# chen-bowen/instacart_next_order_recommendation

Hardware: AMD Instinct MI355X
Metric: recommend_qps_top20_49k7_catalog (higher is better)
Workload: dtype f16x3 (f32 operands split into 2 f16 planes, 3 f16 MFMAs per product, f32 accumulate; fp32-level accuracy)

## Files before the change

### instacart_next_order_recommendation_amd/csrc/encoder.hip

```cpp
#include <stdlib.h>

#include <mutex>
#include <type_traits>
#include <vector>

#include "common.h"
#include "gemm_x3.h"
#include "wt_gemm.h"
#include "encoder_x3.h"

namespace icrec {

__device__ __forceinline__ int find_seq(const int32_t* __restrict__ cu, int n_seqs, int t) {
    int lo = 0, hi = n_seqs;
    while (hi - lo > 1) {
        int mid = (lo + hi) >> 1;
        if (cu[mid] <= t) lo = mid; else hi = mid;
    }
    return lo;
}

template <int H, bool SPLIT>
__device__ __forceinline__ void ln_row(float (&v)[H / 64], const float* __restrict__ g, const float* __restrict__ b,
                                       float eps, float* __restrict__ out, _Float16* __restrict__ oh,
                                       _Float16* __restrict__ ol, int lane) {
    float s = 0.0f;
#pragma unroll
    for (int j = 0; j < H / 64; ++j) s = s + v[j];
    const float mean = wave_sum_f32(s) / (float)H;
    float q = 0.0f;
#pragma unroll
    for (int j = 0; j < H / 64; ++j) {
        float d = v[j] - mean;
        q = fmaf(d, d, q);
    }
    const float var = wave_sum_f32(q) / (float)H;
    const float rstd = 1.0f / sqrtf(var + eps);
#pragma unroll
    for (int j = 0; j < H / 64; ++j) {
        const int i = lane + 64 * j;
        const float y = fmaf((v[j] - mean) * rstd, g[i], b[i]);
        if (SPLIT) {
            _Float16 hi, lo;
            split_act(y, hi, lo);
            oh[i] = hi;
            ol[i] = lo;
        } else {
            out[i] = y;
        }
    }
}

template <int H, bool SPLIT>
__global__ __launch_bounds__(256) void embed_ln_kernel(const int32_t* __restrict__ ids,
                                                       const int32_t* __restrict__ cu, int n_seqs, int T,
                                                       const float* __restrict__ word, const float* __restrict__ pos,
                                                       const float* __restrict__ type, const float* __restrict__ g,
                                                       const float* __restrict__ b, float eps, int vocab, int max_pos,
                                                       float* __restrict__ x, _Float16* __restrict__ xh,
                                                       _Float16* __restrict__ xl) {
    const int lane = threadIdx.x & 63;
    const int t = blockIdx.x * 4 + (threadIdx.x >> 6);
    if (t >= T) return;
    const int s = find_seq(cu, n_seqs, t);
    int id = ids[t];
    id = id < 0 ? 0 : (id >= vocab ? vocab - 1 : id);
    int p = t - cu[s];
    p = p >= max_pos ? max_pos - 1 : p;
    float v[H / 64];
#pragma unroll
    for (int j = 0; j < H / 64; ++j) {
        const int i = lane + 64 * j;
        v[j] = (word[(size_t)id * H + i] + type[i]) + pos[(size_t)p * H + i];
    }
    ln_row<H, SPLIT>(v, g, b, eps, x + (size_t)t * H, xh + (size_t)t * H, xl + (size_t)t * H, lane);
}

template <int H, bool SPLIT>
__global__ __launch_bounds__(256) void add_ln_kernel(const float* __restrict__ a, float* __restrict__ x, int T,
                                                     const float* __restrict__ g, const float* __restrict__ b,
                                                     float eps, _Float16* __restrict__ xh,
                                                     _Float16* __restrict__ xl) {
    const int lane = threadIdx.x & 63;
    const int t = blockIdx.x * 4 + (threadIdx.x >> 6);
    if (t >= T) return;
    float v[H / 64];
#pragma unroll
    for (int j = 0; j < H / 64; ++j) {
        const int i = lane + 64 * j;
        v[j] = a[(size_t)t * H + i] + x[(size_t)t * H + i];
    }
    ln_row<H, SPLIT>(v, g, b, eps, x + (size_t)t * H, xh + (size_t)t * H, xl + (size_t)t * H, lane);
}

__device__ __forceinline__ float gelu_erf(float x) { return x * 0.5f * (1.0f + erff(x * 0.70710678118654752440f)); }

template <class Cfg, bool GELU>
__global__ __launch_bounds__(Cfg::THREADS, 2) void linear_kernel(const float* __restrict__ A, int M, int K,
                                                                 const float* __restrict__ W, int N,
                                                                 const float* __restrict__ bias,
                                                                 float* __restrict__ out, int n_tiles_n) {
    __shared__ __attribute__((aligned(16))) float smem[Cfg::LDS_FLOATS];
    float* As = smem;
    float* Bs = smem + Cfg::BM * LDK;
    const int lane = threadIdx.x & 63, wave = threadIdx.x >> 6;
    const int wm = wave / Cfg::WAVES_N, wn = wave % Cfg::WAVES_N;
    const int bid = xcd_remap(blockIdx.x, gridDim.x);
    const int mt = bid / n_tiles_n, nt = bid % n_tiles_n;
    const int64_t m0 = (int64_t)mt * Cfg::BM, n0 = (int64_t)nt * Cfg::BN;
    TileRegs<Cfg> pre;
    f32x16 acc[Cfg::TM][Cfg::TN];
    tile_gemm<Cfg>(acc, A, m0, M, W, n0, N, K, As, Bs, pre, false);
#pragma unroll
    for (int j = 0; j < Cfg::TN; ++j) {
        const int64_t col = n0 + (wn * Cfg::TN + j) * 32 + (lane & 31);
        const float bv = col < N ? bias[col] : 0.0f;
#pragma unroll
        for (int i = 0; i < Cfg::TM; ++i)
#pragma unroll
            for (int e = 0; e < 16; ++e) {
                const int64_t row = m0 + (wm * Cfg::TM + i) * 32 + acc_row(e, lane);
                if (row < M && col < N) {
                    float v = acc[i][j][e] + bv;
                    if (GELU) v = gelu_erf(v);
                    out[row * N + col] = v;
                }
            }
    }
}

constexpr int DH = 32;
constexpr int LDQ = 36;

template <int NKT, int WAVES, bool SPLIT>
__global__ __launch_bounds__(WAVES * 64) void attention_kernel(const float* __restrict__ qkv,
                                                               const int32_t* __restrict__ cu, int heads, int H,
                                                               float scale_log2e, float* __restrict__ ctx,
                                                               _Float16* __restrict__ ch, _Float16* __restrict__ cl) {
    __shared__ __attribute__((aligned(16))) float Ks[NKT * 32 * LDQ];
    __shared__ __attribute__((aligned(16))) float Vs[NKT * 32 * DH];
    __shared__ float Ls[WAVES * 32];

    const int tid = threadIdx.x, lane = tid & 63, wave = tid >> 6;
    const int s = blockIdx.x / heads, hd = blockIdx.x % heads;
    const int t0 = cu[s], L = cu[s + 1] - t0;
    const int nkt = (L + 31) >> 5;
    if (nkt > NKT || (NKT > 1 && nkt <= NKT / 2)) return;
    const int qb0 = blockIdx.y * WAVES;
    if (qb0 >= nkt) return;
    const int ld = 3 * H;

    for (int id = tid; id < nkt * 32 * 8; id += WAVES * 64) {
        const int row = id >> 3, c = id & 7;
        const int rr = row < L ? row : L - 1;
        const float* src = qkv + (size_t)(t0 + rr) * ld + hd * DH + c * 4;
        const float4 kv = *reinterpret_cast<const float4*>(src + H);
        const float4 vv = *reinterpret_cast<const float4*>(src + 2 * H);
        float* kp = Ks + row * LDQ + (c >> 1) * 8 + (c & 1) * 2;
        *reinterpret_cast<float2*>(kp) = make_float2(kv.x, kv.z);
        *reinterpret_cast<float2*>(kp + 4) = make_float2(kv.y, kv.w);
        *reinterpret_cast<float4*>(Vs + row * DH + c * 4) = vv;
    }
    const int r = lane & 31, h = lane >> 5;
    const int qb = qb0 + wave;
    float4 qf[4];
    {
        int qr = qb * 32 + r;
        qr = qr < L ? qr : L - 1;
        const float4* qp = reinterpret_cast<const float4*>(qkv + (size_t)(t0 + qr) * ld + hd * DH);
#pragma unroll
        for (int kq = 0; kq < 4; ++kq) {
            const float4 a = qp[2 * kq], b = qp[2 * kq + 1];
            qf[kq] = h == 0 ? make_float4(a.x, a.z, b.x, b.z) : make_float4(a.y, a.w, b.y, b.w);
        }
    }
    __syncthreads();
    if (qb >= nkt) return;

    f32x16 sc[NKT];
#pragma unroll
    for (int kt = 0; kt < NKT; ++kt) {
#pragma unroll
        for (int e = 0; e < 16; ++e) sc[kt][e] = 0.0f;
        if (kt < nkt) {
#pragma unroll
            for (int kq = 0; kq < 4; ++kq) {
                const float4 kf = *reinterpret_cast<const float4*>(Ks + (kt * 32 + r) * LDQ + kq * 8 + h * 4);
                sc[kt] = __builtin_amdgcn_mfma_f32_32x32x2f32(kf.x, qf[kq].x, sc[kt], 0, 0, 0);
                sc[kt] = __builtin_amdgcn_mfma_f32_32x32x2f32(kf.y, qf[kq].y, sc[kt], 0, 0, 0);
                sc[kt] = __builtin_amdgcn_mfma_f32_32x32x2f32(kf.z, qf[kq].z, sc[kt], 0, 0, 0);
                sc[kt] = __builtin_amdgcn_mfma_f32_32x32x2f32(kf.w, qf[kq].w, sc[kt], 0, 0, 0);
            }
        }
    }
    float mx = -INFINITY;
#pragma unroll
    for (int kt = 0; kt < NKT; ++kt) {
        if (kt < nkt) {
            const bool last = kt == nkt - 1;
#pragma unroll
            for (int e = 0; e < 16; ++e) {
                float v = sc[kt][e] * scale_log2e;
                if (last && kt * 32 + acc_row(e, lane) >= L) v = -INFINITY;
                sc[kt][e] = v;
                mx = fmaxf(mx, v);
            }
        }
    }
    mx = fmaxf(mx, __shfl_xor(mx, 32, 64));
    float lsum = 0.0f;
#pragma unroll
    for (int kt = 0; kt < NKT; ++kt) {
        if (kt < nkt) {
#pragma unroll
            for (int e = 0; e < 16; ++e) {
                const float p = __builtin_amdgcn_exp2f(sc[kt][e] - mx);
                sc[kt][e] = p;
                lsum = lsum + p;
            }
        }
    }
    {
        const float other = __shfl_xor(lsum, 32, 64);
        lsum = h == 0 ? lsum + other : other + lsum;
    }
    if (h == 0) Ls[wave * 32 + r] = lsum;
    f32x16 o;
#pragma unroll
    for (int e = 0; e < 16; ++e) o[e] = 0.0f;
#pragma unroll
    for (int kt = 0; kt < NKT; ++kt) {
        if (kt < nkt) {
#pragma unroll
            for (int e = 0; e < 16; ++e) {
                const int key = kt * 32 + (e & 3) + 8 * (e >> 2) + 4 * h;
                o = __builtin_amdgcn_mfma_f32_32x32x2f32(sc[kt][e], Vs[key * DH + r], o, 0, 0, 0);
            }
        }
    }
#pragma unroll
    for (int e = 0; e < 16; ++e) {
        const int qrow = acc_row(e, lane);
        const int tq = qb * 32 + qrow;
        if (tq < L) {
            const float v = o[e] / Ls[wave * 32 + qrow];
            const size_t at = (size_t)(t0 + tq) * H + hd * DH + r;
            if (SPLIT) {
                _Float16 hi, lo;
                split_act(v, hi, lo);
                ch[at] = hi;
                cl[at] = lo;
            } else {
                ctx[at] = v;
            }
        }
    }
}

__global__ __launch_bounds__(1024) void seq_order_kernel(const int32_t* __restrict__ cu, int n_seqs,
                                                         int32_t* __restrict__ order) {
    __shared__ int hist[257];
    const int tid = threadIdx.x;
    for (int i = tid; i < 257; i += 1024) hist[i] = 0;
    __syncthreads();
    for (int s0 = tid; s0 < n_seqs; s0 += 1024) {
        const int s = n_seqs - 1 - s0;
        int L = cu[s + 1] - cu[s];
        L = L < 1 ? 1 : (L > 256 ? 256 : L);
        atomicAdd(&hist[256 - ((L + 31) & ~31)], 1);
    }
    __syncthreads();
    if (tid == 0) {
        int run = 0;
        for (int b = 0; b < 257; ++b) { const int c = hist[b]; hist[b] = run; run += c; }
    }
    __syncthreads();
    for (int s0 = tid; s0 < n_seqs; s0 += 1024) {
        const int s = n_seqs - 1 - s0;
        int L = cu[s + 1] - cu[s];
        L = L < 1 ? 1 : (L > 256 ? 256 : L);
        order[atomicAdd(&hist[256 - ((L + 31) & ~31)], 1)] = s;
    }
}

typedef _Float16 half2v __attribute__((ext_vector_type(2)));

__device__ __forceinline__ void split8(const float (&x)[8], half8& hi, half8& lo) {
#pragma unroll
    for (int j = 0; j < 8; ++j) {
        const _Float16 a = (_Float16)x[j];
        hi[j] = a;
        lo[j] = (_Float16)((x[j] - (float)a) * LO_SCALE);
    }
}

__device__ __forceinline__ half4 lds_read_tr(const _Float16* p) {
    typedef __fp16 fp16x4 __attribute__((__vector_size__(4 * sizeof(__fp16))));
    return __builtin_bit_cast(half4, __builtin_amdgcn_ds_read_tr16_b64_v4f16(
                                         (__attribute__((address_space(3))) fp16x4*)(reinterpret_cast<uintptr_t>(p))));
}

template <int NKT, int WAVES, bool SPLIT>
__global__ __launch_bounds__(WAVES * 64, (NKT >= 6 ? 4 : NKT == 4 ? 3 : 1)) void attention_x3_kernel(const float* __restrict__ qkv,
                                                                  const int32_t* __restrict__ cu, int heads, int H,
                                                                  float scale_log2e, float* __restrict__ ctx,
                                                                  _Float16* __restrict__ ch, _Float16* __restrict__ cl,
                                                                  const int32_t* __restrict__ order, int nlo) {
    constexpr bool RECOMP = NKT >= 6;
    __shared__ __attribute__((aligned(16))) _Float16 Kbuf[2 * NKT * 32 * 32];
    _Float16* const Kh = Kbuf;
    _Float16* const Kl = Kbuf + NKT * 32 * 32;
    __shared__ __attribute__((aligned(16))) _Float16 Vh[NKT * 32 * 32];
    __shared__ __attribute__((aligned(16))) _Float16 Vl[NKT * 32 * 32];
    __shared__ float Ls[WAVES * 32];
    constexpr bool OB = SPLIT;
    static_assert(!OB || WAVES * 2 * 32 * 32 <= 2 * NKT * 32 * 32, "the output tiles reuse the K planes");
    _Float16* const Ob = Kbuf;

    const int tid = threadIdx.x, lane = tid & 63, wave = tid >> 6;
    const int sidx = blockIdx.x / heads, hd = blockIdx.x % heads;
    const int s = order != nullptr ? order[sidx] : sidx;
    const int t0 = cu[s], L = cu[s + 1] - t0;
    const int nkt = (L + 31) >> 5;
    if (nkt > NKT || nkt <= nlo) return;
    const int qb0 = blockIdx.y * WAVES;
    if (qb0 >= nkt) return;
    const int ld = 3 * H;

    const int r = lane & 31, h = lane >> 5;
    const int qb = qb0 + wave;
    ICREC_STAMP(0, 0);
    half8 qh[2], ql[2];
    {
        int qr = qb * 32 + r;
        qr = qr < L ? qr : L - 1;
        const float* qp = qkv + (size_t)(t0 + qr) * ld + hd * DH;
#pragma unroll
        for (int ks = 0; ks < 2; ++ks) {
            const f32x4 a = *reinterpret_cast<const f32x4*>(qp + 16 * ks + 8 * h);
            const f32x4 b = *reinterpret_cast<const f32x4*>(qp + 16 * ks + 8 * h + 4);
            half4 ah, al, bh, bl;
            split_act4(a, ah, al);
            split_act4(b, bh, bl);
            qh[ks] = half8{ah[0], ah[1], ah[2], ah[3], bh[0], bh[1], bh[2], bh[3]};
            ql[ks] = half8{al[0], al[1], al[2], al[3], bl[0], bl[1], bl[2], bl[3]};
        }
    }
    ICREC_STAMP(0, 6);
    constexpr int STG = NKT * 32 * 8 / (WAVES * 64);
    static_assert(NKT * 32 * 8 % (WAVES * 64) == 0, "staging: whole rounds");
    f32x4 kreg[STG], vreg[STG];
#pragma unroll
    for (int it = 0; it < STG; ++it) {
        const int id = tid + it * WAVES * 64;
        const int key = id >> 3, c = id & 7;
        const int rr = key < L ? key : L - 1;
        const float* src = qkv + (size_t)(t0 + rr) * ld + hd * DH + c * 4;
        kreg[it] = *reinterpret_cast<const f32x4*>(src + H);
        vreg[it] = *reinterpret_cast<const f32x4*>(src + 2 * H);
    }
#ifdef ICREC_STAMPS
    asm volatile("s_waitcnt vmcnt(0)" ::: "memory");
    ICREC_STAMP(0, 7);
#endif
#pragma unroll
    for (int it = 0; it < STG; ++it) {
        const int id = tid + it * WAVES * 64;
        if (id < nkt * 32 * 8) {
            const int key = id >> 3, c = id & 7;
            half4 khi, klo, vhi, vlo;
            split_act4(kreg[it], khi, klo);
            split_act4(vreg[it], vhi, vlo);
            *reinterpret_cast<half4*>(Vh + key * 32 + c * 4) = vhi;
            *reinterpret_cast<half4*>(Vl + key * 32 + c * 4) = vlo;
            const int off = key * 32 + ((((c >> 1) ^ ((key >> 2) & 3)) << 3) | ((c & 1) << 2));
            *reinterpret_cast<half4*>(Kh + off) = khi;
            *reinterpret_cast<half4*>(Kl + off) = klo;
        }
    }
    ICREC_STAMP(0, 1);
    __syncthreads();
    ICREC_STAMP(0, 2);
    const bool active = qb < nkt;
    if (!RECOMP && !OB && !active) return;

    auto score_tile = [&](int kt, bool hi_only = false) {
        f32x16 t;
#pragma unroll
        for (int e = 0; e < 16; ++e) t[e] = 0.0f;
        const int key = kt * 32 + r;
#pragma unroll
        for (int ks = 0; ks < 2; ++ks) {
            const int off = key * 32 + (((2 * ks + h) ^ ((key >> 2) & 3)) << 3);
            const half8 kh = *reinterpret_cast<const half8*>(Kh + off);
            const half8 kl = *reinterpret_cast<const half8*>(Kl + off);
            t = __builtin_amdgcn_mfma_f32_32x32x16_f16(kh, qh[ks], t, 0, 0, 0);
            if (hi_only) continue;
            t = __builtin_amdgcn_mfma_f32_32x32x16_f16(kh, ql[ks], t, 0, 0, 0);
            t = __builtin_amdgcn_mfma_f32_32x32x16_f16(kl, qh[ks], t, 0, 0, 0);
        }
        if (kt == nkt - 1 && kt * 32 + 32 > L) {
#pragma unroll
            for (int e = 0; e < 16; ++e)
                if (kt * 32 + acc_row(e, lane) >= L) t[e] = -INFINITY;
        }
        return t;
    };
    auto pv_tile = [&](int kt, const f32x16& pt, f32x16& o) {
#pragma unroll
        for (int ks = 0; ks < 2; ++ks) {
            half8 ph, pl;
#pragma unroll
            for (int j = 0; j < 8; j += 2) {
                half2w a, b;
#if defined(ICREC_ATT_ABL) && (ICREC_ATT_ABL & 1)
                a = __builtin_bit_cast(half2w, __builtin_amdgcn_cvt_pkrtz(pt[8 * ks + j], pt[8 * ks + j + 1]));
                b = a;
#else
                split_pair_prescaled(pt[8 * ks + j], pt[8 * ks + j + 1], a, b);
#endif
                ph[j] = a[0]; ph[j + 1] = a[1];
                pl[j] = b[0]; pl[j + 1] = b[1];
            }
            const int base = kt * 32 + 4 * h + 16 * ks;
            const int tr_at = (base + ((lane & 15) >> 2)) * 32 + 16 * ((lane >> 4) & 1) + 4 * (lane & 3);
            const half4 v0h = lds_read_tr(Vh + tr_at);
            const half4 v1h = lds_read_tr(Vh + tr_at + 8 * 32);
            const half4 v0l = lds_read_tr(Vl + tr_at);
            const half4 v1l = lds_read_tr(Vl + tr_at + 8 * 32);
            const half8 vh = {v0h[0], v0h[1], v0h[2], v0h[3], v1h[0], v1h[1], v1h[2], v1h[3]};
            const half8 vl = {v0l[0], v0l[1], v0l[2], v0l[3], v1l[0], v1l[1], v1l[2], v1l[3]};
            o = __builtin_amdgcn_mfma_f32_32x32x16_f16(ph, vh, o, 0, 0, 0);
            o = __builtin_amdgcn_mfma_f32_32x32x16_f16(ph, vl, o, 0, 0, 0);
            o = __builtin_amdgcn_mfma_f32_32x32x16_f16(pl, vh, o, 0, 0, 0);
        }
    };
    typedef float float2w __attribute__((ext_vector_type(2)));
    const float cs = scale_log2e * (1.0f / 256.0f);
    f32x16 o;
#pragma unroll
    for (int e = 0; e < 16; ++e) o[e] = 0.0f;
    if (RECOMP) {
        if (active) {
            float mx = -INFINITY;
#pragma unroll
            for (int kt = 0; kt < NKT; ++kt) {
                if (kt < nkt) {
                    const f32x16 t = score_tile(kt, true);
#pragma unroll
                    for (int e = 0; e < 16; ++e) mx = fmaxf(mx, t[e]);
                }
            }
            mx = fmaxf(mx, __shfl_xor(mx, 32, 64));
            ICREC_STAMP(0, 9);
            const float shift = fmaf(-mx, cs, 10.0f);
            float2w ls2 = float2w{0.0f, 0.0f};
#pragma unroll
            for (int kt = 0; kt < NKT; ++kt) {
                if (kt < nkt) {
                    f32x16 t = score_tile(kt);
#pragma unroll
#if defined(ICREC_ATT_ABL) && (ICREC_ATT_ABL & 2)
                    for (int e = 0; e < 16; ++e) t[e] = fmaf(t[e], cs, shift);
#else
                    for (int e = 0; e < 16; ++e) t[e] = __builtin_amdgcn_exp2f(fminf(fmaf(t[e], cs, shift), 15.9f));
#endif
#pragma unroll
                    for (int e = 0; e < 16; e += 2) ls2 = ls2 + float2w{t[e], t[e + 1]};
                    pv_tile(kt, t, o);
                }
            }
            float lrow = ls2[0] + ls2[1];
            const float other = __shfl_xor(lrow, 32, 64);
            lrow = h == 0 ? lrow + other : other + lrow;
            if (h == 0) Ls[wave * 32 + r] = lrow;
        }
        ICREC_STAMP(0, 3);
        __syncthreads();
        if (!active) return;
    } else {
    if (active) {
    f32x16 sc[NKT];
#pragma unroll
    for (int kt = 0; kt < NKT; ++kt)
        if (kt < nkt) sc[kt] = score_tile(kt);
    float mx = -INFINITY;
#pragma unroll
    for (int kt = 0; kt < NKT; ++kt) {
        if (kt < nkt) {
#pragma unroll
            for (int e = 0; e < 16; ++e) mx = fmaxf(mx, sc[kt][e]);
        }
    }
    mx = fmaxf(mx, __shfl_xor(mx, 32, 64));
    const float shift = fmaf(-mx, cs, 10.0f);
#pragma unroll
    for (int kt = 0; kt < NKT; ++kt) {
        if (kt < nkt) {
#pragma unroll
            for (int e = 0; e < 16; ++e) sc[kt][e] = __builtin_amdgcn_exp2f(fmaf(sc[kt][e], cs, shift));
        }
    }
    float2w ls2 = float2w{0.0f, 0.0f};
#pragma unroll
    for (int kt = 0; kt < NKT; ++kt) {
        if (kt < nkt) {
#pragma unroll
            for (int e = 0; e < 16; e += 2) ls2 = ls2 + float2w{sc[kt][e], sc[kt][e + 1]};
        }
    }
    float lrow = ls2[0] + ls2[1];
    {
        const float other = __shfl_xor(lrow, 32, 64);
        lrow = h == 0 ? lrow + other : other + lrow;
    }
    if (h == 0) Ls[wave * 32 + r] = lrow;
    ICREC_STAMP(0, 3);

#pragma unroll
    for (int kt = 0; kt < NKT; ++kt)
        if (kt < nkt) pv_tile(kt, sc[kt], o);
    }
    if (OB) {
        __syncthreads();
        if (!active) return;
    }
    }
    ICREC_STAMP(0, 4);
    if (OB) {
        _Float16* ob = Ob + wave * (2 * 32 * 32);
#pragma unroll
        for (int e = 0; e < 16; e += 2) {
            const int q0 = acc_row(e, lane), q1 = acc_row(e + 1, lane);
            const float v0 = o[e] * (0.0625f * __builtin_amdgcn_rcpf(Ls[wave * 32 + q0]));
            const float v1 = o[e + 1] * (0.0625f * __builtin_amdgcn_rcpf(Ls[wave * 32 + q1]));
            half2w hi, lo;
            split_pair_prescaled(v0 * WT_SA, v1 * WT_SA, hi, lo);
            ob[q0 * 32 + r] = hi[0];
            ob[q1 * 32 + r] = hi[1];
            ob[32 * 32 + q0 * 32 + r] = lo[0];
            ob[32 * 32 + q1 * 32 + r] = lo[1];
        }
#pragma unroll
        for (int t = 0; t < 2; ++t) {
            const int id = lane + 64 * t, qrow = id >> 2, c8 = (id & 3) * 8;
            const int tq = qb * 32 + qrow;
            if (tq < L) {
                const size_t at = (size_t)(t0 + tq) * H + hd * DH + c8;
                *reinterpret_cast<u32x4*>(ch + at) = *reinterpret_cast<const u32x4*>(ob + qrow * 32 + c8);
                *reinterpret_cast<u32x4*>(cl + at) = *reinterpret_cast<const u32x4*>(ob + 32 * 32 + qrow * 32 + c8);
            }
        }
    } else {
#pragma unroll
        for (int e = 0; e < 16; ++e) {
            const int qrow = acc_row(e, lane);
            const int tq = qb * 32 + qrow;
            if (tq < L) {
                const float v = o[e] * (0.0625f * __builtin_amdgcn_rcpf(Ls[wave * 32 + qrow]));
                const size_t at = (size_t)(t0 + tq) * H + hd * DH + r;
                if (SPLIT) {
                    _Float16 hi, lo;
                    split_act(v, hi, lo);
                    ch[at] = hi;
                    cl[at] = lo;
                } else {
                    ctx[at] = v;
                }
            }
        }
    }
    ICREC_STAMP(0, 5);
#ifdef ICREC_STAMPS
    if (threadIdx.x == 0) {
        const unsigned hw = __builtin_amdgcn_s_getreg((31 << 11) | (0 << 6) | 4), xcc = __builtin_amdgcn_s_getreg((3 << 11) | (0 << 6) | 20);
        g_stamps[((size_t)blockIdx.x * 2) * 64 + 8] = ((unsigned long long)xcc << 32) | hw;
    }
#endif
}

template <int H, bool PLANES>
__global__ __launch_bounds__(H) void pool_norm_kernel(const float* __restrict__ x, const _Float16* __restrict__ xh,
                                                      const _Float16* __restrict__ xl, const int32_t* __restrict__ cu,
                                                      int n_norm, float* __restrict__ out) {
    auto at = [&](size_t idx) { return PLANES ? ((float)xh[idx] + (float)xl[idx]) * (1.0f / WT_SA) : x[idx]; };
    __shared__ float v[H];
    __shared__ float den_s;
    const int s = blockIdx.x, i = threadIdx.x;
    const int t0 = cu[s], t1 = cu[s + 1];
    float acc = 0.0f;
    int t = t0;
    for (; t + 8 <= t1; t += 8) {
        float v[8];
#pragma unroll
        for (int u = 0; u < 8; ++u) v[u] = at((size_t)(t + u) * H + i);
#pragma unroll
        for (int u = 0; u < 8; ++u) acc = acc + v[u];
    }
    for (; t < t1; ++t) acc = acc + at((size_t)t * H + i);
    float cnt = (float)(t1 - t0);
    cnt = cnt < 1e-9f ? 1e-9f : cnt;
    float val = acc / cnt;
    for (int rep = 0; rep < n_norm; ++rep) {
        v[i] = val;
        __syncthreads();
        if (i < 64) {
            float a = 0.0f;
#pragma unroll
            for (int j = 0; j < H / 64; ++j) a = fmaf(v[i + 64 * j], v[i + 64 * j], a);
            const float nrm = sqrtf(wave_sum_f32(a));
            if (i == 0) den_s = nrm > 1e-12f ? nrm : 1e-12f;
        }
        __syncthreads();
        val = val / den_s;
        __syncthreads();
    }
    out[(size_t)s * H + i] = val;
}

constexpr int HID = 384;

struct LayerW {
    float *Wqkv, *bqkv, *Wo, *bo, *g1, *b1n, *W1, *b1, *W2, *b2, *g2, *b2n;
    _Float16 *Wqkv_p, *Wo_p, *W1_p, *W2_p;
};
struct Encoder {
    icrec_bert_cfg cfg;
    int device = 0;
    int n_cu = 256;
    float* blob = nullptr;
    float* extra = nullptr;
    _Float16* planes = nullptr;
    float *word, *pos, *type, *eg, *eb;
    LayerW layers[64];
    bool fuse = true, side_stream = true;
    int small_m = 3584;
    int tail_m = 2560;
    struct Side {
        hipStream_t caller = nullptr, side = nullptr;
        hipEvent_t ev_main = nullptr, ev_qkv_tail = nullptr, ev_att = nullptr, ev_tail = nullptr, ev_q = nullptr, ev_sa = nullptr;
    };
    std::mutex side_mu;
    std::vector<Side*> sides;
};

static int side_for(Encoder* e, hipStream_t caller, Encoder::Side** out) {
    std::lock_guard<std::mutex> lock(e->side_mu);
    *out = nullptr;
    for (Encoder::Side* sd : e->sides)
        if (sd->caller == caller) { *out = sd; return ICREC_OK; }
    hipStreamCaptureStatus cap = hipStreamCaptureStatusNone;
    if (caller && hipStreamIsCapturing(caller, &cap) == hipSuccess && cap != hipStreamCaptureStatusNone)
        return ICREC_OK;
    Encoder::Side* sd = new Encoder::Side();
    sd->caller = caller;
    ICREC_HIP(hipStreamCreateWithFlags(&sd->side, hipStreamNonBlocking));
    for (hipEvent_t* ev : {&sd->ev_main, &sd->ev_qkv_tail, &sd->ev_att, &sd->ev_tail, &sd->ev_q, &sd->ev_sa})
        ICREC_HIP(hipEventCreateWithFlags(ev, hipEventDisableTiming));
    e->sides.push_back(sd);
    *out = sd;
    return ICREC_OK;
}

static size_t weight_count(const icrec_bert_cfg* c) {
    const size_t H = c->hidden, I = c->intermediate;
    const size_t emb = (size_t)c->vocab_size * H + (size_t)c->max_position * H + (size_t)c->type_vocab * H + 2 * H;
    const size_t per = 4 * (H * H + H) + 2 * H + (I * H + I) + (H * I + H) + 2 * H;
    return emb + per * c->layers;
}

struct EncWs {
    size_t x, xs, qkv, ctx, t1, h, total;
};
static EncWs enc_ws(const icrec_bert_cfg& c, int64_t T) {
    auto al = [](size_t b) { return (b + 255) & ~(size_t)255; };
    EncWs w;
    size_t o = 0;
    w.x = o;   o += al((size_t)T * c.hidden * 4);
    w.xs = o;  o += al((size_t)T * c.hidden * 4);
    w.qkv = o; o += al((size_t)T * 3 * c.hidden * 4);
    w.ctx = o; o += al((size_t)T * c.hidden * 4);
    w.t1 = o;  o += al((size_t)T * c.hidden * 4);
    w.h = o;   o += al((size_t)T * c.intermediate * 4);
    w.total = o;
    return w;
}

typedef TileCfg<2, 2, 2, 2> GemmBig;
constexpr long long SMALL_M_MAX = 1 << 20;

static int env_knob(const char* name, int fallback, long long hi) {
    const char* s = getenv(name);
    if (!s) return fallback;
    char* end = nullptr;
    const long long v = strtoll(s, &end, 10);
    if (end == s) return fallback;
    return (int)(v < 0 ? 0 : v > hi ? hi : v);
}

template <bool GELU>
static void launch_linear(const float* A, int M, int K, const float* W, int N, const float* bias, float* out,
                          hipStream_t st) {
    const int mt = (M + GemmBig::BM - 1) / GemmBig::BM, nt = (N + GemmBig::BN - 1) / GemmBig::BN;
    hipLaunchKernelGGL((linear_kernel<GemmBig, GELU>), dim3(mt * nt), dim3(GemmBig::THREADS), 0, st, A, M, K, W, N,
                       bias, out, nt);
}

template <int EPI>
static void launch_wt_linear(const _Float16* Xh, const _Float16* Xl, int T, int K, const _Float16* Wp, int N,
                             const float* bias, float* out, _Float16* oh, _Float16* ol, hipStream_t st, int small_m) {
    if (T <= small_m) {
        if constexpr (EPI == 0 || EPI == 2) {
            if (N % 64 == 0 && K % 128 == 0) {
                const int nbn = N / 64;
                if (K % 256 == 0 && K >= 1024)
                    hipLaunchKernelGGL((wt_linear_half_kernel<EPI, 8>), dim3(((T + 31) / 32) * nbn), dim3(256), 0, st, Xh, Xl, T, K, Wp,
                                       N, bias, out, (const _Float16*)oh, (const _Float16*)ol, nbn);
                else if (K % 384 == 0)
                    hipLaunchKernelGGL((wt_linear_half_kernel<EPI, 6>), dim3(((T + 31) / 32) * nbn), dim3(256), 0, st, Xh, Xl, T, K, Wp,
                                       N, bias, out, (const _Float16*)oh, (const _Float16*)ol, nbn);
                else
                hipLaunchKernelGGL((wt_linear_half_kernel<EPI>), dim3(((T + 31) / 32) * nbn), dim3(256), 0, st, Xh, Xl, T, K, Wp, N,
                                   bias, out, (const _Float16*)oh, (const _Float16*)ol, nbn);
                return;
            }
        }
        const int nbn = N / 128;
        hipLaunchKernelGGL((wt_linear_kernel<1, 1, 4, EPI>), dim3(((T + 31) / 32) * nbn), dim3(256), 0, st, Xh, Xl, T, K,
                           Wp, N, bias, out, oh, ol, nbn);
    } else {
        const int nbn = N / 384;
        hipLaunchKernelGGL((wt_linear_kernel<3, 2, 1, EPI>), dim3(((T + 63) / 64) * nbn), dim3(256), 0, st, Xh, Xl, T, K,
                           Wp, N, bias, out, oh, ol, nbn);
    }
}

template <bool SPLIT, bool X3>
static void launch_attention(const float* qkv, const int32_t* cu, int n_seqs, int heads, int H, int max_seqlen,
                             float* ctx, _Float16* ch, _Float16* cl, hipStream_t st, int buckets = 31,
                             const int32_t* order = nullptr) {
    const float sl2e = (1.0f / sqrtf((float)DH)) * 1.44269504088896340736f;
    const int nkt_max = (max_seqlen + 31) / 32;
    const bool single = n_seqs == 1;
    const dim3 grid1(n_seqs * heads, 1);
#define ICREC_ATT(NKT, W, NLO)                                                                                   \
    do {                                                                                                         \
        if (X3) hipLaunchKernelGGL((attention_x3_kernel<NKT, W, SPLIT>), grid1, dim3(W * 64), 0, st, qkv, cu, heads, H, sl2e, ctx, ch, cl, order, NLO); \
        else hipLaunchKernelGGL((attention_kernel<NKT, W, SPLIT>), grid1, dim3(W * 64), 0, st, qkv, cu, heads, H, sl2e, ctx, ch, cl);      \
    } while (0)
    if ((buckets & 1) && (single ? nkt_max == 1 : true)) ICREC_ATT(1, 1, 0);
    if ((buckets & 2) && (single ? nkt_max == 2 : nkt_max >= 2)) ICREC_ATT(2, 2, 1);
    if ((buckets & 4) && (single ? (nkt_max == 3 || nkt_max == 4) : nkt_max >= 3)) ICREC_ATT(4, 4, 2);
    if (X3 && !single) {
        if ((buckets & 8) && nkt_max >= 5) ICREC_ATT(6, 6, 4);
        if ((buckets & 16) && nkt_max >= 7) ICREC_ATT(8, 8, 6);
    } else if ((buckets & 8) && nkt_max >= 5) {
        ICREC_ATT(8, 8, 4);
    }
#undef ICREC_ATT
}

}

using namespace icrec;

extern "C" {

size_t icrec_encoder_weight_count(const icrec_bert_cfg* cfg) { return cfg ? weight_count(cfg) : 0; }

int icrec_encoder_create(const float* weights_host, size_t n_floats, const icrec_bert_cfg* cfg, int device,
                         icrec_encoder** out) {
    ICREC_REQUIRE(weights_host && cfg && out, "icrec_encoder_create: NULL argument");
    ICREC_REQUIRE(cfg->hidden == HID, "icrec_encoder_create: this build supports hidden=384 only (got %d)", cfg->hidden);
    ICREC_REQUIRE(cfg->heads * DH == cfg->hidden, "icrec_encoder_create: head_dim must be 32 (heads=%d)", cfg->heads);
    ICREC_REQUIRE(cfg->intermediate >= 384 && cfg->intermediate % 384 == 0, "icrec_encoder_create: intermediate size must be a multiple of 384 (got %d)", cfg->intermediate);
    ICREC_REQUIRE(cfg->layers >= 1 && cfg->layers <= 64, "icrec_encoder_create: layers must be in [1,64]");
    ICREC_REQUIRE(cfg->vocab_size >= 1 && cfg->max_position >= 1 && cfg->type_vocab >= 1, "icrec_encoder_create: bad vocab/position sizes");
    ICREC_REQUIRE(cfg->n_normalize >= 0 && cfg->n_normalize <= 4, "icrec_encoder_create: n_normalize must be in [0,4]");
    ICREC_REQUIRE(cfg->gemm_mode == ICREC_GEMM_F32 || cfg->gemm_mode == ICREC_GEMM_F16X3, "icrec_encoder_create: unknown gemm_mode %d", cfg->gemm_mode);
    ICREC_REQUIRE(n_floats == weight_count(cfg), "icrec_encoder_create: weight blob has %zu floats, expected %zu", n_floats, weight_count(cfg));
    ICREC_HIP(hipSetDevice(device));
    hipDeviceProp_t prop;
    ICREC_HIP(hipGetDeviceProperties(&prop, device));
    if (strncmp(prop.gcnArchName, "gfx950", 6) != 0) {
        set_error("icrec_encoder_create: device %d is %s, this library is built for gfx950 only", device, prop.gcnArchName);
        return ICREC_ENODEV;
    }
    Encoder* e = new Encoder();
    e->cfg = *cfg;
    e->device = device;
    e->n_cu = prop.multiProcessorCount > 0 ? prop.multiProcessorCount : 256;
    {
        const char* fuse_env = getenv("ICREC_FUSE");
        const char* side_env = getenv("ICREC_SIDE_STREAM");
        e->fuse = !(fuse_env && fuse_env[0] == '0');
        e->small_m = env_knob("ICREC_SMALL_M", e->small_m, SMALL_M_MAX);
        e->tail_m = env_knob("ICREC_TAIL_M", e->tail_m, 64LL * e->n_cu - 1);
        e->side_stream = !(side_env && side_env[0] == '0');
    }
    const size_t H = cfg->hidden, I = cfg->intermediate;
    const size_t mat_per_layer = 3 * H * H + H * H + I * H + H * I;
    const bool x3 = cfg->gemm_mode == ICREC_GEMM_F16X3;
    if (hipMalloc(&e->blob, n_floats * 4) != hipSuccess ||
        hipMalloc(&e->extra, (size_t)cfg->layers * (3 * H * H + 3 * H) * 4) != hipSuccess ||
        (x3 && hipMalloc(&e->planes, (size_t)cfg->layers * mat_per_layer * 2 * sizeof(_Float16)) != hipSuccess)) {
        set_error("icrec_encoder_create: hipMalloc failed");
        if (e->blob) (void)hipFree(e->blob);
        if (e->extra) (void)hipFree(e->extra);
        delete e;
        return ICREC_ENOMEM;
    }
    ICREC_HIP(hipMemcpy(e->blob, weights_host, n_floats * 4, hipMemcpyHostToDevice));
    float* p = e->blob;
    e->word = p; p += (size_t)cfg->vocab_size * H;
    e->pos = p;  p += (size_t)cfg->max_position * H;
    e->type = p; p += (size_t)cfg->type_vocab * H;
    e->eg = p;   p += H;
    e->eb = p;   p += H;
    float* x = e->extra;
    _Float16* pl = e->planes;
    auto pack = [&](const float* w, int N, int K, _Float16*& out) {
        out = pl;
        pl += (size_t)2 * N * K;
        hipLaunchKernelGGL(pack_weights_kernel, dim3(1024), dim3(256), 0, 0, w, N, K, out);
    };
    for (int l = 0; l < cfg->layers; ++l) {
        LayerW& L = e->layers[l];
        L.Wqkv = x; x += 3 * H * H;
        L.bqkv = x; x += 3 * H;
        for (int part = 0; part < 3; ++part) {
            ICREC_HIP(hipMemcpy(L.Wqkv + part * H * H, p, H * H * 4, hipMemcpyDeviceToDevice)); p += H * H;
            ICREC_HIP(hipMemcpy(L.bqkv + part * H, p, H * 4, hipMemcpyDeviceToDevice)); p += H;
        }
        L.Wo = p; p += H * H; L.bo = p; p += H;
        L.g1 = p; p += H; L.b1n = p; p += H;
        L.W1 = p; p += I * H; L.b1 = p; p += I;
        L.W2 = p; p += H * I; L.b2 = p; p += H;
        L.g2 = p; p += H; L.b2n = p; p += H;
        if (x3) {
            pack(L.Wqkv, (int)(3 * H), (int)H, L.Wqkv_p);
            pack(L.Wo, (int)H, (int)H, L.Wo_p);
            pack(L.W1, (int)I, (int)H, L.W1_p);
            pack(L.W2, (int)H, (int)I, L.W2_p);
        }
    }
    ICREC_HIP(hipGetLastError());
    ICREC_HIP(hipDeviceSynchronize());
    *out = reinterpret_cast<icrec_encoder*>(e);
    return ICREC_OK;
}

int icrec_encoder_destroy(icrec_encoder* h) {
    Encoder* e = reinterpret_cast<Encoder*>(h);
    if (!e) return ICREC_OK;
    (void)hipSetDevice(e->device);
    (void)hipFree(e->blob);
    (void)hipFree(e->extra);
    if (e->planes) (void)hipFree(e->planes);
    for (Encoder::Side* sd : e->sides) {
        if (sd->side) {
            (void)hipStreamSynchronize(sd->side);
            (void)hipStreamDestroy(sd->side);
        }
        for (hipEvent_t ev : {sd->ev_main, sd->ev_qkv_tail, sd->ev_att, sd->ev_tail, sd->ev_q, sd->ev_sa})
            if (ev) (void)hipEventDestroy(ev);
        delete sd;
    }
    delete e;
    return ICREC_OK;
}

size_t icrec_encode_workspace_bytes(const icrec_encoder* h, int64_t total_tokens, int32_t n_seqs) {
    const Encoder* e = reinterpret_cast<const Encoder*>(h);
    if (!e || total_tokens < 1 || n_seqs < 1) return 0;
    return enc_ws(e->cfg, total_tokens).total;
}

static void batch_split(const Encoder* e, int T, int* t_main, int* t_tail) {
    const int round_tokens = 64 * e->n_cu;
    *t_main = T;
    *t_tail = 0;
    if (T > round_tokens && T % round_tokens != 0 && T % round_tokens <= e->tail_m) {
        *t_tail = T % round_tokens;
        *t_main = T - *t_tail;
    }
}

int icrec_encode_batch_split(const icrec_encoder* h, int64_t total_tokens, int64_t* main_tokens, int64_t* tail_tokens) {
    const Encoder* e = reinterpret_cast<const Encoder*>(h);
    ICREC_REQUIRE(e && main_tokens && tail_tokens && total_tokens >= 1 && total_tokens < (1ll << 31), "icrec_encode_batch_split: bad argument");
    int m, t;
    batch_split(e, (int)total_tokens, &m, &t);
    *main_tokens = m;
    *tail_tokens = t;
    return ICREC_OK;
}

int icrec_encode(icrec_encoder* h, const int32_t* ids_dev, const int32_t* cu_dev, int32_t n_seqs, int64_t T64,
                 int32_t max_seqlen, float* out_dev, void* ws, size_t ws_bytes, void* stream) {
    Encoder* e = reinterpret_cast<Encoder*>(h);
    ICREC_REQUIRE(e && ids_dev && cu_dev && out_dev, "icrec_encode: NULL argument");
    ICREC_REQUIRE(n_seqs >= 1 && T64 >= n_seqs && T64 < (1ll << 31), "icrec_encode: bad n_seqs/total_tokens (%d, %lld)", n_seqs, (long long)T64);
    ICREC_REQUIRE(max_seqlen >= 1 && max_seqlen <= 256 && max_seqlen <= e->cfg.max_position, "icrec_encode: max_seqlen must be in [1, 256] (got %d)", max_seqlen);
    const int T = (int)T64;
    const EncWs w = enc_ws(e->cfg, T);
    if (!ws || ws_bytes < w.total) {
        set_error("icrec_encode: workspace too small (%zu < %zu)", ws_bytes, w.total);
        return ICREC_ENOMEM;
    }
    ICREC_HIP(hipSetDevice(e->device));
    hipStream_t st = (hipStream_t)stream;
    ScopedTimer whole(T_ENCODE, st);
    char* base = reinterpret_cast<char*>(ws);
    float* x = reinterpret_cast<float*>(base + w.x);
    float* qkv = reinterpret_cast<float*>(base + w.qkv);
    float* ctx = reinterpret_cast<float*>(base + w.ctx);
    float* t1 = reinterpret_cast<float*>(base + w.t1);
    float* hb = reinterpret_cast<float*>(base + w.h);
    const icrec_bert_cfg& c = e->cfg;
    const int H = c.hidden, I = c.intermediate;
    const int rows_grid = (T + 3) / 4;
    const bool x3 = c.gemm_mode == ICREC_GEMM_F16X3;
    int T_main, T_tail;
    batch_split(e, T, &T_main, &T_tail);
    const bool fuse = e->fuse, side_stream = e->side_stream;
    const int small_m = e->small_m;
    const bool qkv_res = fuse && H == 384;
    const bool lnin = fuse && H == 384 && I % 64 == 0;
    const bool split_att = x3 && side_stream && n_seqs >= 64 && max_seqlen > 128;
    Encoder::Side* sd = nullptr;
    if (x3 && side_stream && (T_tail || split_att))
        if (int rc_ = side_for(e, st, &sd)) return rc_;
    const bool use_side = sd != nullptr;
    _Float16* xh = reinterpret_cast<_Float16*>(base + w.xs);
    _Float16* xl = xh + (size_t)T * H;
    _Float16* ch = reinterpret_cast<_Float16*>(ctx);
    _Float16* cl = ch + (size_t)T * H;
    _Float16* hh = reinterpret_cast<_Float16*>(hb);
    _Float16* hl = hh + (size_t)T * I;

    const int32_t* order = nullptr;
    if (x3 && n_seqs >= 64 && fuse) {
        int32_t* ord = reinterpret_cast<int32_t*>(x);
        hipLaunchKernelGGL(seq_order_kernel, dim3(1), dim3(1024), 0, st, cu_dev, n_seqs, ord);
        order = ord;
    }
    if (x3)
        hipLaunchKernelGGL((embed_ln_kernel<HID, true>), dim3(rows_grid), dim3(256), 0, st, ids_dev, cu_dev, n_seqs, T,
                           e->word, e->pos, e->type, e->eg, e->eb, c.ln_eps, c.vocab_size, c.max_position, x, xh, xl);
    else
        hipLaunchKernelGGL((embed_ln_kernel<HID, false>), dim3(rows_grid), dim3(256), 0, st, ids_dev, cu_dev, n_seqs, T,
                           e->word, e->pos, e->type, e->eg, e->eb, c.ln_eps, c.vocab_size, c.max_position, x, xh, xl);
    for (int l = 0; l < c.layers; ++l) {
        const LayerW& L = e->layers[l];
        if (x3) {
            auto qkv_stage = [&](int r0, int Tn, hipStream_t st) -> int {
                if (Tn > small_m && qkv_res) {
                    auto kern = qkv_resident_kernel;
                    if (int rc_ = ensure_dynamic_lds(reinterpret_cast<const void*>(kern), QKVR_LDS)) return rc_;
                    hipLaunchKernelGGL(kern, dim3((Tn + 63) / 64), dim3(512), QKVR_LDS, st, xh + (size_t)r0 * H,
                                       xl + (size_t)r0 * H, Tn, L.Wqkv_p, L.bqkv, qkv + (size_t)r0 * 3 * H, 3 * H);
                    return ICREC_OK;
                }
                if (lnin && l > 0 && Tn <= small_m) {
                    const LayerW& Lp = e->layers[l - 1];
                    const int nbn = 3 * H / 64;
                    hipLaunchKernelGGL((wt_linear_lnin_kernel<0, true>), dim3(((Tn + 31) / 32) * nbn), dim3(256), 0, st,
                                       (const float*)(t1 + (size_t)r0 * H), Tn, Lp.g2, Lp.b2n, c.ln_eps, xh + (size_t)r0 * H,
                                       xl + (size_t)r0 * H, L.Wqkv_p, 3 * H, L.bqkv, qkv + (size_t)r0 * 3 * H,
                                       (_Float16*)nullptr, (_Float16*)nullptr, nbn);
                    return ICREC_OK;
                }
                launch_wt_linear<0>(xh + (size_t)r0 * H, xl + (size_t)r0 * H, Tn, H, L.Wqkv_p, 3 * H, L.bqkv,
                                    qkv + (size_t)r0 * 3 * H, nullptr, nullptr, st, small_m);
                return ICREC_OK;
            };
            auto post_stage = [&](int r0, int Tn, hipStream_t st) -> int {
                float* const t1r = t1 + (size_t)r0 * H;
                _Float16 *const xhr = xh + (size_t)r0 * H, *const xlr = xl + (size_t)r0 * H;
                const _Float16 *const chr = ch + (size_t)r0 * H, *const clr = cl + (size_t)r0 * H;
                if (Tn > small_m && fuse) {
                    ScopedTimer tm(T_FFN_UP, st);
                    const int nblk = (Tn + 63) / 64;
                    auto kern = ffn_fused2_kernel<0, true>;
                    if (int rc_ = ensure_dynamic_lds(reinterpret_cast<const void*>(kern), FFN2_LDS)) return rc_;
                    const bool next_qkv = l + 1 < c.layers;
                    const LayerW& Ln = e->layers[next_qkv ? l + 1 : l];
                    hipLaunchKernelGGL(kern, dim3(nblk), dim3(512), FFN2_LDS, st, xhr, xlr, Tn, I, L.W1_p, L.b1, L.W2_p,
                                       L.b2, L.g2, L.b2n, c.ln_eps, chr, clr, L.Wo_p, L.bo, L.g1, L.b1n,
                                       next_qkv ? (const _Float16*)Ln.Wqkv_p : (const _Float16*)nullptr, (const float*)Ln.bqkv,
                                       qkv + (size_t)r0 * 3 * H, 3 * H);
                } else {
                    _Float16 *const hhr = hh + (size_t)r0 * I, *const hlr = hl + (size_t)r0 * I;
                    launch_wt_linear<2>(chr, clr, Tn, H, L.Wo_p, H, L.bo, t1r, xhr, xlr, st, small_m);
                    if (lnin && Tn <= small_m) {
                        const int nbn = I / 64;
                        hipLaunchKernelGGL((wt_linear_lnin_kernel<1, true>), dim3(((Tn + 31) / 32) * nbn), dim3(256), 0, st,
                                           (const float*)t1r, Tn, L.g1, L.b1n, c.ln_eps, xhr, xlr, L.W1_p, I, L.b1,
                                           (float*)nullptr, hhr, hlr, nbn);
                    } else {
                    hipLaunchKernelGGL(ln_wt_kernel, dim3((Tn + 15) / 16), dim3(256), 0, st, t1r, Tn, L.g1, L.b1n,
                                       c.ln_eps, xhr, xlr);
                    {
                        ScopedTimer tm(Tn > small_m ? T_FFN_UP : T_NSLOTS - 1, st);
                        launch_wt_linear<1>(xhr, xlr, Tn, H, L.W1_p, I, L.b1, nullptr, hhr, hlr, st, small_m);
                    }
                    }
                    launch_wt_linear<2>(hhr, hlr, Tn, I, L.W2_p, H, L.b2, t1r, xhr, xlr, st, small_m);
                    if (!(lnin && Tn <= small_m && l + 1 < c.layers))
                    hipLaunchKernelGGL(ln_wt_kernel, dim3((Tn + 15) / 16), dim3(256), 0, st, t1r, Tn, L.g2, L.b2n,
                                       c.ln_eps, xhr, xlr);
                }
                return ICREC_OK;
            };
            const bool qkv_in_fused = fuse && T_main > small_m && H == 384;
            const bool tail_qkv_in_fused = fuse && T_tail > small_m && H == 384;
            hipStream_t ts = st;
            if (T_tail && use_side) {
                ts = sd->side;
                if (l == 0) {
                    ICREC_HIP(hipEventRecord(sd->ev_main, st));
                    ICREC_HIP(hipStreamWaitEvent(ts, sd->ev_main, 0));
                }
                if (l == 0 || !tail_qkv_in_fused)
                    if (int rc_ = qkv_stage(T_main, T_tail, ts)) return rc_;
                ICREC_HIP(hipEventRecord(sd->ev_qkv_tail, ts));
            } else if (T_tail && (l == 0 || !tail_qkv_in_fused)) {
                if (int rc_ = qkv_stage(T_main, T_tail, st)) return rc_;
            }
            if (l == 0 || !qkv_in_fused)
                if (int rc_ = qkv_stage(0, T_main, st)) return rc_;
            if (T_tail && use_side) ICREC_HIP(hipStreamWaitEvent(st, sd->ev_qkv_tail, 0));
            if (split_att && use_side) {
                ICREC_HIP(hipEventRecord(sd->ev_q, st));
                ICREC_HIP(hipStreamWaitEvent(sd->side, sd->ev_q, 0));
                launch_attention<true, true>(qkv, cu_dev, n_seqs, c.heads, H, max_seqlen, ctx, ch, cl, sd->side, 7 | 16, order);
                ICREC_HIP(hipEventRecord(sd->ev_sa, sd->side));
                launch_attention<true, true>(qkv, cu_dev, n_seqs, c.heads, H, max_seqlen, ctx, ch, cl, st, 8, order);
                ICREC_HIP(hipStreamWaitEvent(st, sd->ev_sa, 0));
            } else {
                launch_attention<true, true>(qkv, cu_dev, n_seqs, c.heads, H, max_seqlen, ctx, ch, cl, st, 31, order);
            }
            if (T_tail) {
                if (use_side) {
                    ICREC_HIP(hipEventRecord(sd->ev_att, st));
                    ICREC_HIP(hipStreamWaitEvent(ts, sd->ev_att, 0));
                }
                if (int rc_ = post_stage(T_main, T_tail, ts)) return rc_;
            }
            if (int rc_ = post_stage(0, T_main, st)) return rc_;
            if (T_tail && use_side && l + 1 == c.layers) {
                ICREC_HIP(hipEventRecord(sd->ev_tail, ts));
                ICREC_HIP(hipStreamWaitEvent(st, sd->ev_tail, 0));
            }
        } else {
            launch_linear<false>(x, T, H, L.Wqkv, 3 * H, L.bqkv, qkv, st);
            launch_attention<false, false>(qkv, cu_dev, n_seqs, c.heads, H, max_seqlen, ctx, ch, cl, st);
            launch_linear<false>(ctx, T, H, L.Wo, H, L.bo, t1, st);
            hipLaunchKernelGGL((add_ln_kernel<HID, false>), dim3(rows_grid), dim3(256), 0, st, t1, x, T, L.g1, L.b1n,
                               c.ln_eps, xh, xl);
            {
                ScopedTimer tm(T_FFN_UP, st);
                launch_linear<true>(x, T, H, L.W1, I, L.b1, hb, st);
            }
            launch_linear<false>(hb, T, I, L.W2, H, L.b2, t1, st);
            hipLaunchKernelGGL((add_ln_kernel<HID, false>), dim3(rows_grid), dim3(256), 0, st, t1, x, T, L.g2, L.b2n,
                               c.ln_eps, xh, xl);
        }
    }
    if (x3) hipLaunchKernelGGL((pool_norm_kernel<HID, true>), dim3(n_seqs), dim3(HID), 0, st, x, xh, xl, cu_dev, c.n_normalize, out_dev);
    else hipLaunchKernelGGL((pool_norm_kernel<HID, false>), dim3(n_seqs), dim3(HID), 0, st, x, xh, xl, cu_dev, c.n_normalize, out_dev);
    ICREC_HIP(hipGetLastError());
    return ICREC_OK;
}

}
```

Measured before the change: 109,400.

## Add persistent work-stealing attention kernel over length-sorted sequence-head items

Adds a persistent attention kernel, launched with two blocks per CU, that pulls sequence-head work items from a global atomic counter. Long sequences (more than 128 tokens) get a full 8-wave block, and pairs of short sequences share a block in two 4-wave halves. The sort kernel now also writes the long-sequence count and zeroes one counter per layer. This replaces the per-length-class launches and the side-stream split attention, aiming to cut launch count and load imbalance. The cost is one atomic per item and fixed barrier counts for skipped items, which must match the barriers inside the item routine.

```diff
diff --git a/instacart_next_order_recommendation_amd/csrc/encoder.hip b/instacart_next_order_recommendation_amd/csrc/encoder.hip
--- a/instacart_next_order_recommendation_amd/csrc/encoder.hip
+++ b/instacart_next_order_recommendation_amd/csrc/encoder.hip
@@ -258,7 +258,7 @@
 }
 
 __global__ __launch_bounds__(1024) void seq_order_kernel(const int32_t* __restrict__ cu, int n_seqs,
-                                                         int32_t* __restrict__ order) {
+                                                         int32_t* __restrict__ order, int n_counters) {
     __shared__ int hist[257];
     const int tid = threadIdx.x;
     for (int i = tid; i < 257; i += 1024) hist[i] = 0;
@@ -273,7 +273,9 @@
     if (tid == 0) {
         int run = 0;
         for (int b = 0; b < 257; ++b) { const int c = hist[b]; hist[b] = run; run += c; }
-    }
+        order[n_seqs] = hist[128];
+    }
+    for (int i = tid; i < n_counters; i += 1024) order[n_seqs + 1 + i] = 0;
     __syncthreads();
     for (int s0 = tid; s0 < n_seqs; s0 += 1024) {
         const int s = n_seqs - 1 - s0;
@@ -300,31 +302,21 @@
                                          (__attribute__((address_space(3))) fp16x4*)(reinterpret_cast<uintptr_t>(p))));
 }
 
+constexpr int ATT_X3_BARRIERS = 2;
 template <int NKT, int WAVES, bool SPLIT>
-__global__ __launch_bounds__(WAVES * 64, (NKT >= 6 ? 4 : NKT == 4 ? 3 : 1)) void attention_x3_kernel(const float* __restrict__ qkv,
-                                                                  const int32_t* __restrict__ cu, int heads, int H,
-                                                                  float scale_log2e, float* __restrict__ ctx,
-                                                                  _Float16* __restrict__ ch, _Float16* __restrict__ cl,
-                                                                  const int32_t* __restrict__ order, int nlo) {
+__device__ __forceinline__ void attention_x3_item(const float* __restrict__ qkv, int t0, int L, int hd, int H,
+                                                  float scale_log2e, float* __restrict__ ctx, _Float16* __restrict__ ch,
+                                                  _Float16* __restrict__ cl, _Float16* Kbuf, _Float16* Vh, _Float16* Vl,
+                                                  float* Ls, int tid, int qb0) {
     constexpr bool RECOMP = NKT >= 6;
-    __shared__ __attribute__((aligned(16))) _Float16 Kbuf[2 * NKT * 32 * 32];
     _Float16* const Kh = Kbuf;
     _Float16* const Kl = Kbuf + NKT * 32 * 32;
-    __shared__ __attribute__((aligned(16))) _Float16 Vh[NKT * 32 * 32];
-    __shared__ __attribute__((aligned(16))) _Float16 Vl[NKT * 32 * 32];
-    __shared__ float Ls[WAVES * 32];
     constexpr bool OB = SPLIT;
     static_assert(!OB || WAVES * 2 * 32 * 32 <= 2 * NKT * 32 * 32, "the output tiles reuse the K planes");
     _Float16* const Ob = Kbuf;
 
-    const int tid = threadIdx.x, lane = tid & 63, wave = tid >> 6;
-    const int sidx = blockIdx.x / heads, hd = blockIdx.x % heads;
-    const int s = order != nullptr ? order[sidx] : sidx;
-    const int t0 = cu[s], L = cu[s + 1] - t0;
+    const int lane = tid & 63, wave = tid >> 6;
     const int nkt = (L + 31) >> 5;
-    if (nkt > NKT || nkt <= nlo) return;
-    const int qb0 = blockIdx.y * WAVES;
-    if (qb0 >= nkt) return;
     const int ld = 3 * H;
 
     const int r = lane & 31, h = lane >> 5;
@@ -579,6 +571,69 @@
 #endif
 }
 
+template <int NKT, int WAVES, bool SPLIT>
+__global__ __launch_bounds__(WAVES * 64, (NKT >= 6 ? 4 : NKT == 4 ? 3 : 1)) void attention_x3_kernel(const float* __restrict__ qkv,
+                                                                  const int32_t* __restrict__ cu, int heads, int H,
+                                                                  float scale_log2e, float* __restrict__ ctx,
+                                                                  _Float16* __restrict__ ch, _Float16* __restrict__ cl,
+                                                                  const int32_t* __restrict__ order, int nlo) {
+    __shared__ __attribute__((aligned(16))) _Float16 Kbuf[2 * NKT * 32 * 32];
+    __shared__ __attribute__((aligned(16))) _Float16 Vh[NKT * 32 * 32];
+    __shared__ __attribute__((aligned(16))) _Float16 Vl[NKT * 32 * 32];
+    __shared__ float Ls[WAVES * 32];
+    const int sidx = blockIdx.x / heads, hd = blockIdx.x % heads;
+    const int s = order != nullptr ? order[sidx] : sidx;
+    const int t0 = cu[s], L = cu[s + 1] - t0;
+    const int nkt = (L + 31) >> 5;
+    if (nkt > NKT || nkt <= nlo) return;
+    const int qb0 = blockIdx.y * WAVES;
+    if (qb0 >= nkt) return;
+    attention_x3_item<NKT, WAVES, SPLIT>(qkv, t0, L, hd, H, scale_log2e, ctx, ch, cl, Kbuf, Vh, Vl, Ls, threadIdx.x, qb0);
+}
+
+template <bool SPLIT>
+__global__ __launch_bounds__(512, 4) void attention_x3_persist_kernel(const float* __restrict__ qkv,
+                                                                     const int32_t* __restrict__ cu, int n_seqs, int heads,
+                                                                     int H, float scale_log2e, float* __restrict__ ctx,
+                                                                     _Float16* __restrict__ ch, _Float16* __restrict__ cl,
+                                                                     const int32_t* __restrict__ meta, int* __restrict__ counter) {
+    __shared__ __attribute__((aligned(16))) _Float16 Kbuf[2 * 8 * 32 * 32];
+    __shared__ __attribute__((aligned(16))) _Float16 Vh[8 * 32 * 32];
+    __shared__ __attribute__((aligned(16))) _Float16 Vl[8 * 32 * 32];
+    __shared__ float Ls[8 * 32];
+    __shared__ int item_s[2];
+    const int n_units = n_seqs * heads, n_long = meta[n_seqs] * heads;
+    const int n_items = n_long + (n_units - n_long + 1) / 2;
+    if (threadIdx.x == 0) item_s[0] = atomicAdd(counter, 1);
+    for (int par = 0;; par ^= 1) {
+        __syncthreads();
+        const int item = item_s[par];
+        if (item >= n_items) break;
+        if (threadIdx.x == 0) item_s[par ^ 1] = atomicAdd(counter, 1);
+        int tid = threadIdx.x;
+        asm volatile("" : "+v"(tid));
+        if (item < n_long) {
+            const int s = meta[item / heads], hd = item % heads;
+            const int t0 = cu[s], L = cu[s + 1] - t0;
+            if (L <= 8 * 32)
+                attention_x3_item<8, 8, SPLIT>(qkv, t0, L, hd, H, scale_log2e, ctx, ch, cl, Kbuf, Vh, Vl, Ls, tid, 0);
+            else
+                for (int b = 0; b < ATT_X3_BARRIERS; ++b) __syncthreads();
+        } else {
+            const int half = tid >> 8;
+            const int unit = n_long + 2 * (item - n_long) + half;
+            const int s = unit < n_units ? meta[unit / heads] : 0, hd = unit % heads;
+            const int t0 = cu[s], L = unit < n_units ? cu[s + 1] - t0 : 0;
+            if (L >= 1 && L <= 4 * 32)
+                attention_x3_item<4, 4, SPLIT>(qkv, t0, L, hd, H, scale_log2e, ctx, ch, cl, Kbuf + half * (2 * 4 * 32 * 32),
+                                               Vh + half * (4 * 32 * 32), Vl + half * (4 * 32 * 32), Ls + half * (4 * 32),
+                                               tid & 255, 0);
+            else
+                for (int b = 0; b < ATT_X3_BARRIERS; ++b) __syncthreads();
+        }
+    }
+}
+
 template <int H, bool PLANES>
 __global__ __launch_bounds__(H) void pool_norm_kernel(const float* __restrict__ x, const _Float16* __restrict__ xh,
                                                       const _Float16* __restrict__ xl, const int32_t* __restrict__ cu,
@@ -633,7 +688,7 @@
     _Float16* planes = nullptr;
     float *word, *pos, *type, *eg, *eb;
     LayerW layers[64];
-    bool fuse = true, side_stream = true;
+    bool fuse = true, side_stream = true, att_persist = true;
     int small_m = 3584;
     int tail_m = 2560;
     struct Side {
@@ -760,6 +815,15 @@
 #undef ICREC_ATT
 }
 
+template <bool SPLIT>
+static void launch_attention_persist(const float* qkv, const int32_t* cu, int n_seqs, int heads, int H, float* ctx,
+                                     _Float16* ch, _Float16* cl, const int32_t* meta, int* counter, int n_cu,
+                                     hipStream_t st) {
+    const float sl2e = (1.0f / sqrtf((float)DH)) * 1.44269504088896340736f;
+    hipLaunchKernelGGL((attention_x3_persist_kernel<SPLIT>), dim3(2 * n_cu), dim3(512), 0, st, qkv, cu, n_seqs, heads, H,
+                       sl2e, ctx, ch, cl, meta, counter);
+}
+
 }
 
 using namespace icrec;
@@ -793,6 +857,8 @@
     {
         const char* fuse_env = getenv("ICREC_FUSE");
         const char* side_env = getenv("ICREC_SIDE_STREAM");
+        const char* persist_env = getenv("ICREC_ATT_PERSIST");
+        e->att_persist = !(persist_env && persist_env[0] == '0');
         e->fuse = !(fuse_env && fuse_env[0] == '0');
         e->small_m = env_knob("ICREC_SMALL_M", e->small_m, SMALL_M_MAX);
         e->tail_m = env_knob("ICREC_TAIL_M", e->tail_m, 64LL * e->n_cu - 1);
@@ -927,7 +993,9 @@
     const int small_m = e->small_m;
     const bool qkv_res = fuse && H == 384;
     const bool lnin = fuse && H == 384 && I % 64 == 0;
-    const bool split_att = x3 && side_stream && n_seqs >= 64 && max_seqlen > 128;
+    const bool batch_order = x3 && n_seqs >= 64 && fuse;
+    const bool persist_att = batch_order && e->att_persist;
+    const bool split_att = x3 && side_stream && n_seqs >= 64 && max_seqlen > 128 && !persist_att;
     Encoder::Side* sd = nullptr;
     if (x3 && side_stream && (T_tail || split_att))
         if (int rc_ = side_for(e, st, &sd)) return rc_;
@@ -940,10 +1008,12 @@
     _Float16* hl = hh + (size_t)T * I;
 
     const int32_t* order = nullptr;
-    if (x3 && n_seqs >= 64 && fuse) {
+    int* att_counters = nullptr;
+    if (batch_order) {
         int32_t* ord = reinterpret_cast<int32_t*>(x);
-        hipLaunchKernelGGL(seq_order_kernel, dim3(1), dim3(1024), 0, st, cu_dev, n_seqs, ord);
+        hipLaunchKernelGGL(seq_order_kernel, dim3(1), dim3(1024), 0, st, cu_dev, n_seqs, ord, persist_att ? c.layers : 0);
         order = ord;
+        att_counters = ord + n_seqs + 1;
     }
     if (x3)
         hipLaunchKernelGGL((embed_ln_kernel<HID, true>), dim3(rows_grid), dim3(256), 0, st, ids_dev, cu_dev, n_seqs, T,
@@ -1038,6 +1108,8 @@
                 ICREC_HIP(hipEventRecord(sd->ev_sa, sd->side));
                 launch_attention<true, true>(qkv, cu_dev, n_seqs, c.heads, H, max_seqlen, ctx, ch, cl, st, 8, order);
                 ICREC_HIP(hipStreamWaitEvent(st, sd->ev_sa, 0));
+            } else if (persist_att) {
+                launch_attention_persist<true>(qkv, cu_dev, n_seqs, c.heads, H, ctx, ch, cl, order, att_counters + l, e->n_cu, st);
             } else {
                 launch_attention<true, true>(qkv, cu_dev, n_seqs, c.heads, H, max_seqlen, ctx, ch, cl, st, 31, order);
             }
```

After: 110,400 (median of 6 runs). No clear change (+0.9%).
